# nikopj/FluxMPI.jl

Hardware: AMD Instinct MI355X
Metric: images/sec ResNet50 Lux.jl DDP at 1/2/4/8 MI355X; scaling efficiency (higher is better)
Workload: dtype bf16; 1 GPU; model=ResNet50, global_batch=256, per_gpu_batch=256, image_size=224, parallelism=dp1, optimizer=adam, conv=hybrid, norm=fused, memory_format=channels_last, backend=rccl, miopen_find=True, hip_graph=False, tunableop=False, kernel_choices=shipped, loss_finite=True, communicate=False

## Files before the change

csrc/api.h:

```cpp
#pragma once
#include <hip/hip_runtime.h>
#include <cstdint>
#include <vector>

namespace fluxmpi {

void mt_copy(const std::vector<uintptr_t>& src, const std::vector<uintptr_t>& dst,
             const std::vector<int64_t>& numel, int in_dtype, int out_dtype, float scale,
             hipStream_t stream);

void mt_fill(const std::vector<uintptr_t>& dst, const std::vector<int64_t>& numel, int dtype,
             float value, hipStream_t stream);

void mt_sumsq(const std::vector<uintptr_t>& src, const std::vector<int64_t>& numel, int dtype,
              float* out, hipStream_t stream);

struct AdamHyper {
  float lr, beta1, beta2, eps;
  float bc1, bc2;
  float weight_decay;
  float grad_scale;
  const float* dev;
  const float* dev_gscale;
  const void* tscale = nullptr;
// ... 123 lines not shown
                  int wdtype, hipStream_t stream, bool colsum);

struct GemmProblem {
  const void* a;
  const void* b;
  void* c;
  int64_t lda, ldb, ldc, M, N, K;
  bool a_kmajor, b_kmajor;
  int mode, splits;
  const float* a_scale;
  const float* a_shift;
  const float* b_scale;
  const float* b_shift;
  float* stats;
  int tile_m, tile_n;
  int nbuf;
  const void* res;
  int64_t ldr;
  const void* bnb_x;
  const float* bnb_w;
  const float* bnb_b;
  const float* bnb_mean;
  const float* bnb_inv;
  const uint8_t* bnb_mask;
  int bnb_rm;
  int conv_h = 0, conv_w = 0, conv_c = 0;
  int engine = 0;
  const uint8_t* res_mask = nullptr;
  int res_sub_h = 0, res_sub_w = 0;
  int a_sub_h = 0, a_sub_w = 0;
  int conv_s = 1;
};
void gemm_bf16(const GemmProblem& g, hipStream_t stream);
bool gemm_glds_supported(const GemmProblem& g);
void gemm_glds(const GemmProblem& g, hipStream_t stream);
void gemm_wgrad(const void* a, const void* b, float* ws, int64_t lda, int64_t ldb, int64_t M, int64_t N, int64_t K,
                int splits, int conv_h, int conv_w, int conv_c, hipStream_t stream, int variant = 0, int b_sub = 0);
void transpose_filters(const std::vector<uintptr_t>& src, const std::vector<uintptr_t>& dst,
                       const std::vector<int>& co, const std::vector<int>& ci, const std::vector<int>& taps,
                       hipStream_t stream);
void gemm_splitk_reduce(const float* ws, int splits, int64_t n, void* out, int out_dtype, hipStream_t stream);
void gemm_splitk_reduce_seg(const float* ws, int splits, int64_t n, int64_t seg, void* out0, void* out1, void* out2,
                            int out_dtype, hipStream_t stream);
bool wgrad256_supported(int64_t M, int64_t N, int64_t K, int64_t lda, int64_t ldb);
int wgrad256_actual_splits(int64_t K, int splits);
void wgrad256_set_variant(int v);
void gemm_wgrad256(const void* a, const void* b, float* ws, int64_t lda, int64_t ldb, int64_t M, int64_t N, int64_t K,
                   int splits, hipStream_t stream);
bool gemm_nt_supported(int64_t M, int64_t N, int64_t K, int64_t lda, int64_t ldb, int64_t ldc);
bool gemm_nt_conv_supported(int64_t pixels, int64_t C, int64_t Cout);
int gemm_nt_colpart_rows(int64_t M);
void gemm_nt_set_split(int min_ktiles);
int gemm_nt_get_split();
void gemm_nt(const void* a, const void* b, void* c, void* c2, const void* bias, int bias_f32, const void* h,
             float* colpart, float* stats, int64_t lda, int64_t ldb, int64_t ldc, int64_t M, int64_t N, int64_t K,
             int epi, hipStream_t stream);
void gemm_nt_conv(const void* x, const void* w, void* y, float* stats, int64_t nimg, int H, int W, int C,
                  int64_t Cout, int epi, hipStream_t stream, const void* residual = nullptr);
bool linear_bwd_supported(int64_t M, int64_t N, int64_t K, int64_t ldy, int64_t ldx, int64_t ldw, int64_t lddx);
int linear_bwd_splits(int64_t M, int64_t N, int64_t K, int splits);
void linear_bwd(const void* dy, const void* x, const void* w, void* dx, float* ws, int64_t M, int64_t N, int64_t K,
                int64_t ldy, int64_t ldx, int64_t ldw, int64_t lddx, int splits, int dg_first, hipStream_t stream);
bool conv_c3_supported(int64_t N, int H, int W, int stride, int Cout);
int64_t conv_c3_wgrad_blocks(int64_t N, int H, int W, int stride);
void conv_c3_fwd(const void* x, const void* w_pairs, void* y, int64_t N, int H, int W, int stride, int Cout,
                 hipStream_t stream);
// ... 57 lines not shown
```

csrc/kernels/batchnorm.hip:

```cpp
#include <cstdlib>
#include <initializer_list>
#include <stdexcept>
#include <string>

#include "../api.h"
#include "common.h"

namespace fluxmpi {
namespace {

constexpr int kThreads = 256;
constexpr int kMaxC = 2048;

template <typename T>
struct V8 {
  T v[8];
};

template <typename T>
__device__ __forceinline__ void ld8f(const T* __restrict__ p, float (&f)[8]) {
  T t[8];
  load8(p, t);
#pragma unroll
  for (int j = 0; j < 8; ++j) f[j] = static_cast<float>(t[j]);
}

template <typename T>
__device__ __forceinline__ void st8f(T* __restrict__ p, const float (&f)[8]) {
  T t[8];
#pragma unroll
  for (int j = 0; j < 8; ++j) t[j] = static_cast<T>(f[j]);
  store8(p, t);
}

__device__ __forceinline__ void ld8ch(const float* __restrict__ p, int c0, float (&v)[8]) {
  const float4 a = *reinterpret_cast<const float4*>(p + c0);
  const float4 b = *reinterpret_cast<const float4*>(p + c0 + 4);
  v[0] = a.x; v[1] = a.y; v[2] = a.z; v[3] = a.w;
// ... 445 lines not shown
      for (int u = 0; u < U; ++u)
#pragma unroll
        for (int j = 0; j < 8; ++j) {
          float dd = static_cast<float>(d[u][j]);
          const float xf = static_cast<float>(xv[u][j]);
          if (RM == 1) dd = static_cast<float>(yv[u][j]) > 0.f ? dd : 0.f;
          if (RM == 2) dd = fmaf(xf, sc[j], sh[j]) > 0.f ? dd : 0.f;
          if (RM == 3) dd = (mb[u] >> j) & 1u ? dd : 0.f;
          s[j] += dd;
          q[j] = fmaf(dd, (xf - mu[j]) * is[j], q[j]);
        }
    }
    for (; r < end; r += g.rpi) {
      const int64_t off = r * C + c8 * 8;
      float d[8], xv[8], yv[8];
      ld8f(dy + off, d);
      ld8f(x + off, xv);
      if (RM == 1) ld8f(y + off, yv);
      const unsigned mbs = RM == 3 ? mask[off >> 3] : 0u;
#pragma unroll
      for (int j = 0; j < 8; ++j) {
        float dd = d[j];
        if (RM == 1) dd = yv[j] > 0.f ? dd : 0.f;
        if (RM == 2) dd = fmaf(xv[j], sc[j], sh[j]) > 0.f ? dd : 0.f;
        if (RM == 3) dd = (mbs >> j) & 1u ? dd : 0.f;
        s[j] += dd;
        q[j] = fmaf(dd, (xv[j] - mu[j]) * is[j], q[j]);
      }
    }
  }
  block_reduce<DET>(s, q, g.cv, g.rpi, C, acc, smem);
}

struct DxCoef {
  float a, b, d, sh;
};

__device__ __forceinline__ DxCoef dx_coef(int c, const float* __restrict__ w, const float* __restrict__ bias,
                                          const float* __restrict__ smean, const float* __restrict__ sinv,
                                          const float* __restrict__ dw, const float* __restrict__ db, float inv_n) {
  const float iv = sinv[c], m = smean[c];
  const float sc = (w ? w[c] : 1.f) * iv;
  const float k2 = db[c] * inv_n, k3 = dw[c] * inv_n;
  DxCoef k;
  k.a = sc;
  k.b = -sc * iv * k3;
  k.d = sc * (m * iv * k3 - k2);
  k.sh = fmaf(-m, sc, bias ? bias[c] : 0.f);
  return k;
}

template <typename T, int RM, bool DRES>
__device__ __forceinline__ void dx_vec(float (&d)[8], float (&xv)[8], const float (&yv)[8], unsigned mbs,
                                       const DxCoef* k) {
#pragma unroll
  for (int j = 0; j < 8; ++j) {
    float dd = d[j];
    if (RM == 1) dd = yv[j] > 0.f ? dd : 0.f;
    if (RM == 3) dd = (mbs >> j) & 1u ? dd : 0.f;
    if (RM == 2) dd = fmaf(xv[j], k[j].a, k[j].sh) > 0.f ? dd : 0.f;
    d[j] = dd;
    xv[j] = fmaf(k[j].a, dd, fmaf(k[j].b, xv[j], k[j].d));
  }
}

template <typename T, int RM, bool DRES, bool FIXED, int U = 2>
__global__ __launch_bounds__(kThreads) void bn_bwd_dx_kernel(const T* __restrict__ dy, const T* __restrict__ x,
                                                             const T* __restrict__ y,
                                                             const uint8_t* __restrict__ mask,
                                                             const float* __restrict__ w,
                                                             const float* __restrict__ bias,
                                                             const float* __restrict__ smean,
                                                             const float* __restrict__ sinv,
                                                             const float* __restrict__ dw,
                                                             const float* __restrict__ db, T* __restrict__ dx,
                                                             T* __restrict__ dres, int64_t rows, int C,
                                                             int64_t nvec) {
  extern __shared__ __attribute__((aligned(16))) DxCoef ksm[];
  const float inv_n = 1.f / static_cast<float>(rows);
  DxCoef rk[8];
  if (FIXED) {
    const int c0 = (threadIdx.x % (C / 8)) * 8;
    float iv[8], m[8], ww[8], bb[8], kdb[8], kdw[8];
    ld8ch(sinv, c0, iv);
    ld8ch(smean, c0, m);
    ld8ch(db, c0, kdb);
    ld8ch(dw, c0, kdw);
    ld8ch(w ? w : smean, c0, ww);
    ld8ch(bias ? bias : smean, c0, bb);
#pragma unroll
    for (int j = 0; j < 8; ++j) {
      const float sc = (w ? ww[j] : 1.f) * iv[j];
      const float k2 = kdb[j] * inv_n, k3 = kdw[j] * inv_n;
      rk[j].a = sc;
      rk[j].b = -sc * iv[j] * k3;
      rk[j].d = sc * (m[j] * iv[j] * k3 - k2);
      rk[j].sh = fmaf(-m[j], sc, bias ? bb[j] : 0.f);
    }
  } else {
    for (int c = threadIdx.x; c < C; c += kThreads) ksm[c] = dx_coef(c, w, bias, smean, sinv, dw, db, inv_n);
    __syncthreads();
  }
  const int64_t stride = static_cast<int64_t>(gridDim.x) * kThreads;
  int64_t v = static_cast<int64_t>(blockIdx.x) * kThreads + threadIdx.x;
  for (; v + (U - 1) * stride < nvec; v += U * stride) {
    float d[U][8], xv[U][8], yv[U][8];
    unsigned mb[U];
#pragma unroll
    for (int u = 0; u < U; ++u) {
      const int64_t vu = v + u * stride;
      ld8f(dy + vu * 8, d[u]);
      ld8f(x + vu * 8, xv[u]);
      if (RM == 1) ld8f(y + vu * 8, yv[u]);
      mb[u] = RM == 3 ? mask[vu] : 0u;
    }
    __builtin_amdgcn_sched_barrier(0);
#pragma unroll
    for (int u = 0; u < U; ++u) {
      const int64_t vu = v + u * stride;
      dx_vec<T, RM, DRES>(d[u], xv[u], yv[u], mb[u], FIXED ? rk : ksm + (vu * 8) % C);
      st8f(dx + vu * 8, xv[u]);
      if (DRES) st8f(dres + vu * 8, d[u]);
    }
  }
  for (; v < nvec; v += stride) {
    float d0[8], x0[8], y0[8];
    ld8f(dy + v * 8, d0);
    ld8f(x + v * 8, x0);
    if (RM == 1) ld8f(y + v * 8, y0);
    const unsigned m0 = RM == 3 ? mask[v] : 0u;
    dx_vec<T, RM, DRES>(d0, x0, y0, m0, FIXED ? rk : ksm + (v * 8) % C);
// ... 376 lines not shown
                       int stats_ready, int dtype, hipStream_t s, int64_t* nbt) {
  check(C);
  if (!stats_ready)
    dispatch_float(dtype, kBadDtype, [&](auto tag) { stats_t<typename decltype(tag)::type>(x, ws, rows, C, s); });
  finalize_fwd(ws, rows, C, momentum, eps, sm, si, rm, rv, w, b, scale, shift, nbt, s);
}

void bn_apply(const void* x, void* y, const void* res, const float* w, const float* b, const float* sm,
              const float* si, int64_t rows, int64_t C, int relu, uint8_t* mask, int dtype, hipStream_t s) {
  check(C);
  check_aligned({w, b, sm, si});
  dispatch_float(dtype, kBadDtype, [&](auto tag) {
    norm_t<typename decltype(tag)::type>(x, y, res, w, b, sm, si, rows, C, 0.f, 1, relu, mask, s);
  });
}

void bn_fwd_infer(const void* x, void* y, const void* residual, const float* weight, const float* bias,
                  const float* running_mean, const float* running_var, int64_t rows, int64_t C, float eps, int relu,
                  int dtype, hipStream_t stream) {
  check(C);
  check_aligned({weight, bias, running_mean, running_var});
  dispatch_float(dtype, kBadDtype, [&](auto tag) {
    norm_t<typename decltype(tag)::type>(x, y, residual, weight, bias, running_mean, running_var, rows, C, eps, 0, relu,
                                         nullptr, stream);
  });
}

void bn_bwd(const void* dy, const void* x, const void* y, const uint8_t* relu_mask, const float* weight,
            const float* bias, const float* save_mean,
            const float* save_invstd, void* dx, void* dres, float* dweight, float* dbias, float* workspace,
            int64_t rows, int64_t C, int relu, int dtype, hipStream_t stream, int stats_ready) {
  check(C);
  check_aligned({weight, bias, save_mean, save_invstd, dweight, dbias});
  const int rm = relu_mode(relu, y, relu_mask);
  dispatch_float(dtype, kBadDtype, [&](auto tag) {
    using T = typename decltype(tag)::type;
    if (!stats_ready)
      bwd_reduce_t<T, false>(dy, x, y, relu_mask, weight, bias, save_mean, save_invstd, workspace, rows, C, rm, stream);
    bn_finalize_bwd(workspace, C, dweight, dbias, stream);
    dx_t<T>(dy, x, y, relu_mask, weight, bias, save_mean, save_invstd, dweight, dbias, dx, dres, rows, rows, C, rm,
            stream);
  });
}

size_t bn_sync_workspace_floats(int64_t rows, int64_t C) {
  check(C);
  return static_cast<size_t>(det_geometry(rows, C).blocks) * 2 * static_cast<size_t>(C);
}

void bn_sync_stats(const void* x, float* part, float* msg, int64_t rows, int64_t C, int dtype, hipStream_t stream,
                   float* save_mean, float* save_invstd, float* running_mean, float* running_var, float momentum,
                   float eps, int64_t* nbt) {
  check(C);
  check_rows(rows);
  check_aligned({msg, save_mean, save_invstd});
  const Geo g = det_geometry(rows, C);
  dispatch_float(dtype, kBadSyncDtype, [&](auto tag) {
    using T = typename decltype(tag)::type;
    bn_stats_kernel<T, true><<<g.blocks, kThreads, reduce_smem(g, C), stream>>>(static_cast<const T*>(x), rows, (int)C,
                                                                                g, part);
  });
  FLUXMPI_HIP_CHECK(hipGetLastError());
  bn_sync_fold_fwd_kernel<<<fold_blocks(C), kFoldCh * kFoldGroups, 0, stream>>>(
      part, g.blocks, (int)C, rows, msg, momentum, eps, save_mean, save_invstd, running_mean, running_var, nbt);
  FLUXMPI_HIP_CHECK(hipGetLastError());
}

void bn_sync_finalize_fwd(const float* msg, float* running_mean, float* running_var, float* save_mean,
                          float* save_invstd, int64_t C, float momentum, float eps, hipStream_t stream,
                          int64_t* nbt) {
  check(C);
  check_aligned({save_mean, save_invstd});
// ... 46 lines not shown
```

csrc/kernels/gemm.hip:

```cpp
#include <cstdlib>
#include <stdexcept>
#include <string>

#include "../api.h"
#include "common.h"

namespace fluxmpi {
namespace {

typedef __bf16 bf16x8 __attribute__((ext_vector_type(8)));
typedef __bf16 bf16x4 __attribute__((ext_vector_type(4)));
typedef float f32x4 __attribute__((ext_vector_type(4)));

constexpr int kThreads = 256;
constexpr int BK = 32;
constexpr int kShards = 64;

struct GemmArgs {
  const bf16* a;
  const bf16* b;
  void* c;
  int64_t lda, ldb, ldc;
  int64_t M, N, K;
  int64_t k_per_split;
// ... 497 lines not shown
    o[3] = static_cast<TO>(r.w);
  }
}

template <typename TO>
__global__ __launch_bounds__(kThreads) void sumall_kernel(const float* __restrict__ ws, int S, TO* __restrict__ out) {
  float acc = 0.f;
  for (int i = threadIdx.x; i < S; i += kThreads) acc += ws[i];
  __shared__ float red[kThreads / 64];
  const float w = wave_sum_dpp(acc);
  if ((threadIdx.x & 63) == 0) red[threadIdx.x >> 6] = w;
  __syncthreads();
  if (threadIdx.x == 0) {
    float t = 0.f;
#pragma unroll
    for (int i = 0; i < kThreads / 64; ++i) t += red[i];
    out[0] = static_cast<TO>(t);
  }
}

template <int BM, int BN, bool AK, bool BKM, int NBUF, bool EX = false, bool CONV = false>
void launch(const GemmArgs& a0, int splits, hipStream_t s) {
  GemmArgs a = a0;
  a.tiles_m = static_cast<int>((a.M + BM - 1) / BM);
  a.tiles_n = static_cast<int>((a.N + BN - 1) / BN);
  dim3 grid(a.tiles_m * a.tiles_n, 1, splits);
  gemm_kernel<BM, BN, AK, BKM, NBUF, EX, CONV><<<grid, kThreads, 0, s>>>(a);
  FLUXMPI_HIP_CHECK(hipGetLastError());
}

}

void gemm_bf16(const GemmProblem& g, hipStream_t stream) {
  const bool glds_only = g.res_mask != nullptr || g.res_sub_h > 0 || g.a_sub_h > 0 || g.conv_s == 2 || g.conv_s >= 16;
  if (glds_only && !gemm_glds_supported(g))
    throw std::runtime_error("gemm_bf16: a masked / subsampled residual or a subsampled A needs the LDS-DMA kernel");
  if (g.engine >= 2 || glds_only || (g.engine == 0 && g.a_scale == nullptr && gemm_glds_supported(g))) {
    gemm_glds(g, stream);
    return;
  }
  if ((g.a_kmajor || g.b_kmajor) && g.K % 8 != 0) throw std::runtime_error("gemm_bf16: K-major operands need K % 8 == 0");
  if ((g.a_kmajor ? g.lda : g.lda) % 8 != 0 || g.ldb % 8 != 0)
    throw std::runtime_error("gemm_bf16: leading dimensions must be multiples of 8");
  if (g.mode == 1 && g.stats == nullptr) throw std::runtime_error("gemm_bf16: stats buffer required");
  if ((g.a_scale != nullptr) && !g.a_kmajor) throw std::runtime_error("gemm_bf16: A affine needs K-major A");
  if ((g.b_scale != nullptr) && g.b_kmajor) throw std::runtime_error("gemm_bf16: B affine needs N-major B");
  GemmArgs a{};
  a.a = static_cast<const bf16*>(g.a);
  a.b = static_cast<const bf16*>(g.b);
  a.c = g.c;
  a.lda = g.lda; a.ldb = g.ldb; a.ldc = g.ldc;
  a.M = g.M; a.N = g.N; a.K = g.K;
  int splits = g.splits < 1 ? 1 : g.splits;
  int64_t kps = ((g.K + BK - 1) / BK + splits - 1) / splits * BK;
  splits = static_cast<int>((g.K + kps - 1) / kps);
  a.k_per_split = kps;
  a.a_scale = g.a_scale; a.a_shift = g.a_shift;
  a.b_scale = g.b_scale; a.b_shift = g.b_shift;
  a.stats = g.stats;
  a.mode = g.mode;
  a.res = static_cast<const bf16*>(g.res);
  a.ldr = g.ldr;
  a.bnb_x = static_cast<const bf16*>(g.bnb_x);
  a.bnb_w = g.bnb_w;
  a.bnb_b = g.bnb_b;
  a.bnb_mean = g.bnb_mean;
// ... 118 lines not shown
```

fluxmpi_amd/_build.py:

```python
from __future__ import annotations

import concurrent.futures as cf
import glob
import os
import shutil
import subprocess
import sys
import sysconfig

ROOT = os.path.dirname(os.path.dirname(os.path.abspath(__file__)))
CSRC = os.path.join(ROOT, "csrc")
BUILD = os.path.join(ROOT, "build", "native")
ROCM = os.environ.get("ROCM_PATH", "/opt/rocm")
ARCH = os.environ.get("FLUXMPI_ARCH", "gfx950")


def _ext_suffix() -> str:
    return sysconfig.get_config_var("EXT_SUFFIX") or ".so"


def output_path() -> str:
    return os.path.join(ROOT, "fluxmpi_amd", "_C" + _ext_suffix())


def _sources() -> list[str]:
    srcs = sorted(glob.glob(os.path.join(CSRC, "**", "*.hip"), recursive=True))
    srcs += sorted(glob.glob(os.path.join(CSRC, "**", "*.cpp"), recursive=True))
    return srcs


def _headers() -> list[str]:
    return sorted(glob.glob(os.path.join(CSRC, "**", "*.h"), recursive=True))


def _torch_lib() -> str:
    import importlib.util

    spec = importlib.util.find_spec("torch")
    return os.path.join(os.path.dirname(spec.origin), "lib")


def _tool(name: str) -> str:
    for cand in (os.path.join(ROCM, "bin", name), os.path.join(ROCM, "llvm", "bin", name), shutil.which(name)):
        if cand and os.path.exists(cand):
            return cand
    raise FileNotFoundError(f"{name} not found (ROCM_PATH={ROCM})")


def _obj_for(src: str) -> str:
    rel = os.path.relpath(src, CSRC).replace(os.sep, "__")
    return os.path.join(BUILD, rel + ".o")


_NO_SLP = ["-fno-slp-vectorize"]
EXTRA_FLAGS = {f: _NO_SLP for f in ("gemm_nt.hip", "attention.hip", "gemm_glds.hip", "gemm.hip", "conv3x3n.hip",
                                        "wgrad3x3n.hip", "linbwd.hip")}


def _compile_cmd(src: str, obj: str) -> list[str]:
    import pybind11

    common = ["-O3", "-fPIC", "-std=c++17", "-I", CSRC, "-Wall", "-Wno-unused-function",
              "-Wno-unused-variable", "-Wno-unused-but-set-variable"]
    if src.endswith(".hip"):
        return [_tool("hipcc"), f"--offload-arch={ARCH}", "-c", src, "-o", obj, *common,
                "-munsafe-fp-atomics", *EXTRA_FLAGS.get(os.path.basename(src), [])]
    inc = [f"-I{pybind11.get_include()}", f"-I{sysconfig.get_paths()['include']}", f"-I{ROCM}/include"]
    return [_tool("amdclang++"), "-D__HIP_PLATFORM_AMD__=1", "-c", src, "-o", obj, *common, *inc,
            "-fvisibility=hidden"]


def _stale(obj: str, deps: list[str]) -> bool:
    if not os.path.exists(obj):
        return True
    t = os.path.getmtime(obj)
    return any(os.path.getmtime(d) > t for d in deps)


def build(force: bool = False, verbose: bool = False, jobs: int | None = None) -> str:
    os.makedirs(BUILD, exist_ok=True)
    headers = _headers()
    srcs = _sources()
    out = output_path()
    jobs = jobs or min(8, os.cpu_count() or 4)

    todo = [(s, _obj_for(s)) for s in srcs if force or _stale(_obj_for(s), [s, *headers])]

    def run(cmd):
        if verbose:
            print(" ".join(cmd), flush=True)
        r = subprocess.run(cmd, capture_output=True, text=True)
        if r.returncode != 0:
            raise RuntimeError(f"command failed ({r.returncode}): {' '.join(cmd)}\n{r.stdout}\n{r.stderr}")
        if verbose and (r.stderr.strip()):
            print(r.stderr, file=sys.stderr)
        return r

    with cf.ThreadPoolExecutor(max_workers=jobs) as ex:
        list(ex.map(lambda so: run(_compile_cmd(*so)), todo))

    objs = [_obj_for(s) for s in srcs]
    if force or todo or _stale(out, objs):
        tl = _torch_lib()
        cmd = [_tool("hipcc"), f"--offload-arch={ARCH}", "-shared", "-fPIC", "-o", out + ".tmp", *objs,
               f"-L{ROCM}/lib", "-lamdhip64", f"-L{tl}", "-l:librccl.so", f"-Wl,-rpath,{tl}",
               f"-Wl,-rpath,{ROCM}/lib"]
        run(cmd)
        os.replace(out + ".tmp", out)
    return out


if __name__ == "__main__":
    p = build(force="--force" in sys.argv, verbose=True)
    print(p)
```

fluxmpi_amd/models/resnet.py:

```python
from __future__ import annotations

import os

import torch
import torch.nn as nn
import torch.nn.functional as F

from ..ops.linear import Linear

STEM = os.environ.get("FLUXMPI_STEM", "ours")


class Conv1x1(nn.Module):

    def __init__(self, cin: int, cout: int, stride: int = 1):
        super().__init__()
        self.stride = stride
        self.weight = nn.Parameter(torch.empty(cout, cin, 1, 1))
        nn.init.kaiming_normal_(self.weight, mode="fan_out", nonlinearity="relu")

    def forward(self, x):
        if self.stride != 1:
            x = x[:, :, ::self.stride, ::self.stride]
        n, c, h, w = x.shape
# ... 84 lines not shown
                    a1 = fb.bn_from_stats(c1, self.bn1, relu=True, stats_ready=True) if o1 else \
                        self.bn1(c1, relu=True)
                else:
                    c1 = fb.conv1x1_stats(x, self.conv1.weight, link)
                    a1 = fb.bn_from_stats(c1, self.bn1, relu=True)
                cds = None
                if self.downsample is None:
                    identity = x
                elif fused_ds:
                    ds = self.downsample
                    dual = fb.dual_bn_ok(x, ds[0].out_channels, self.bn3, ds[1])
                    ds_stats = dual and fb.ds_forward_is_ours(x, ds[0].weight, ds[0].stride[0])
                    identity = fb.conv1x1_downsample(x, ds[0].weight, ds[0].stride[0],
                                                     link if isinstance(link, fb.SideGradLink) else None,
                                                     ours_stats=ds_stats)
                    if dual:
                        cds, identity = identity, None
                    else:
                        identity = ds[1](identity)
                else:
                    identity = self.downsample(x)
                if self.hybrid:
                    if fb.conv3x3_supported(a1, self.conv2):
                        ours = fb.conv3x3_forward_is_ours(a1, self.conv2.weight)
                        c2 = fb.conv3x3(a1, self.conv2.weight, with_stats=True)
                        a2 = fb.bn_from_stats(c2, self.bn2, relu=True, stats_ready=ours)
                    elif fb.conv3x3_s2_supported(a1, self.conv2):
                        ours = fb.conv3x3_s2_forward_is_ours(a1, self.conv2.weight)
                        c2 = fb.conv3x3_s2(a1, self.conv2.weight, with_stats=ours)
                        a2 = fb.bn_from_stats(c2, self.bn2, relu=True, stats_ready=ours)
                    else:
                        a2 = self.bn2(self.conv2(a1), relu=True)
                    o3 = fb.conv1x1_forward_is_ours(a2, self.conv3.weight)
                    c3 = fb.conv1x1_hybrid(a2, self.conv3.weight, None, ours_stats=o3)
                else:
                    c2 = fb.conv3x3(a1, self.conv2.weight) if fb.conv3x3_supported(a1, self.conv2) else self.conv2(a1)
                    c3 = fb.bn_relu_conv1x1(c2, self.bn2, self.conv3.weight)
                if cds is not None:
                    out = fb.dual_bn_relu(c3, self.bn3, cds, self.downsample[1],
                                          stats_ready=o3 if self.hybrid else True, ds_stats_ready=ds_stats)
                elif self.hybrid and not o3:
                    out = self.bn3(c3, relu=True, residual=identity, link=link if self.downsample is None else None)
                elif self.hybrid:
                    out = fb.bn_from_stats(c3, self.bn3, relu=True, residual=identity, stats_ready=True,
                                           link=link if self.downsample is None else None)
                else:
                    out = fb.bn_from_stats(c3, self.bn3, relu=True, residual=identity,
                                           link=link if self.downsample is None else None)
                return out
        identity = x if self.downsample is None else self.downsample(x)
        if self.fused:
            out = self.bn1(self.conv1(x), relu=True)
            out = self.bn2(self.conv2(out), relu=True)
            return self.bn3(self.conv3(out), relu=True, residual=identity)
        out = F.relu(self.bn1(self.conv1(x)))
        out = F.relu(self.bn2(self.conv2(out)))
        out = self.bn3(self.conv3(out))
        return F.relu(out + identity)


class ResNet(nn.Module):
    def __init__(self, layers=(3, 4, 6, 3), num_classes=1000, conv_impl="gemm", norm="torch", zero_init_residual=False):
        super().__init__()
        if conv_impl in ("fused", "hybrid"):
            if norm == "sync":
                raise ValueError(f"norm='sync' cannot be combined with conv_impl={conv_impl!r}: those blocks and the "
# ... 79 lines not shown
```

fluxmpi_amd/ops/fused_block.py:

```python
from __future__ import annotations

import torch

from . import _ext
from . import graddst
from .batchnorm import BNStatsLink, GradLink, SideGradLink, _dual_workspace, _link_workspace, _workspace, bn_counter
from . import gemm as G
from . import gemm_nt as _NT
from . import groupnorm as _GN
from .conv_choice import (_DGRAD_CHOICE, _DS_CHOICE, _FWD1_CHOICE, _FWD_CHOICE, _FWD_ENGINE, _S2_CHOICE,
                          _WG_CHOICE, FWD_ENGINES, choices_frozen, dump_choices, freeze_choices,
                          load_choice_lines, load_choices, no_measure as _no_measure, stats_choice,
                          time_us as _time_us, w256_ok as _w256_ok, w3n_configs, wgrad_best)
from .gemm import conv1x1_dgrad, conv1x1_wgrad, conv3x3_dgrad, conv3x3_fwd, gemm, note_filter
from .multi_tensor import DTYPE_CODE


CONV3X3 = "ours"
CONV1X1 = "ours"
DUAL_BN = True
DS_FWD = "ours"
DS_WGRAD = True
S2_FWD = True


def _stream(t):
    return torch.cuda.current_stream(t.device).cuda_stream


def _p(t):
    return t.data_ptr() if t is not None else 0


# ... 246 lines not shown
                            float(eps), int(stats_ready), DTYPE_CODE[x.dtype], _stream(x), _p(nbt))
        res = None
        if residual is not None:
            res = residual if residual.is_contiguous(memory_format=torch.channels_last) else \
                residual.contiguous(memory_format=torch.channels_last)
        y = torch.empty_like(x)
        mask = torch.empty(x.numel() // 8, device=x.device, dtype=torch.uint8) if (relu and res is not None) \
            else None
        C.bn_apply(x.data_ptr(), y.data_ptr(), _p(res), w32.data_ptr(), b32.data_ptr(), mean.data_ptr(),
                   inv.data_ptr(), rows, ch, int(relu), _p(mask), DTYPE_CODE[x.dtype], _stream(x))
        ctx.relu, ctx.has_res, ctx.wdtype = relu, residual is not None, weight.dtype
        ctx.params = (weight, bias)
        ctx.link = link if residual is not None else None
        ctx.bnlink = bnlink
        if bnlink is not None:
            bnlink.bind(x, mask, w32, b32, mean, inv, relu)
        ctx.save_for_backward(x, mask, w32, b32, mean, inv)
        return y

    @staticmethod
    def backward(ctx, dy):
        x, mask, w32, b32, mean, inv = ctx.saved_tensors
        if not dy.is_contiguous(memory_format=torch.channels_last):
            dy = dy.contiguous(memory_format=torch.channels_last)
        ready = ctx.bnlink is not None and ctx.bnlink.ready
        hand_masked = ctx.link is not None and ctx.link.masked and mask is not None and ctx.relu
        dx, dres, dw, db = _bn_bwd(dy, x, mask, w32, b32, mean, inv, ctx.relu, ctx.has_res and not hand_masked,
                                   ready, ctx.params)
        if ctx.bnlink is not None:
            ctx.bnlink.release()
        if ctx.link is not None:
            ctx.link.grad, dres = ((dy, mask) if hand_masked else dres), None
        return dx, dw.to(ctx.wdtype), db.to(ctx.wdtype), dres, None, None, None, None, None, None, None, None, None


class _DualBN(torch.autograd.Function):

    @staticmethod
    def forward(ctx, c3, w, b, rm, rv, mom, eps, nbt, stats_ready, cds, w2, b2, rm2, rv2, mom2, eps2, nbt2,
                ds_ready=False):
        C = _ext.get(required=True)
        cl = torch.channels_last
        c3 = c3 if c3.is_contiguous(memory_format=cl) else c3.contiguous(memory_format=cl)
        cds = cds if cds.is_contiguous(memory_format=cl) else cds.contiguous(memory_format=cl)
        ch = c3.shape[1]
        rows = c3.numel() // ch
        f32 = dict(device=c3.device, dtype=torch.float32)
        w32, b32, w232, b232 = w.float(), b.float(), w2.float(), b2.float()
        mean, inv, mean2, inv2 = (torch.empty(ch, **f32) for _ in range(4))
        ws, code, st = _workspace(c3), DTYPE_CODE[c3.dtype], _stream(c3)
        C.bn_stats_finalize(c3.data_ptr(), w32.data_ptr(), b32.data_ptr(), _p(rm), _p(rv), mean.data_ptr(),
                            inv.data_ptr(), 0, 0, ws.data_ptr(), rows, ch, float(mom), float(eps), int(stats_ready),
                            code, st, _p(nbt))
        ws2 = _dual_workspace(c3) if ds_ready else ws
        C.bn_stats_finalize(cds.data_ptr(), w232.data_ptr(), b232.data_ptr(), _p(rm2), _p(rv2), mean2.data_ptr(),
                            inv2.data_ptr(), 0, 0, ws2.data_ptr(), rows, ch, float(mom2), float(eps2), int(ds_ready),
                            code, st, _p(nbt2))
        y = torch.empty_like(c3)
        mask = torch.empty(c3.numel() // 8, device=c3.device, dtype=torch.uint8)
        C.bn_apply_dual(c3.data_ptr(), cds.data_ptr(), y.data_ptr(), w32.data_ptr(), b32.data_ptr(), mean.data_ptr(),
                        inv.data_ptr(), w232.data_ptr(), b232.data_ptr(), mean2.data_ptr(), inv2.data_ptr(), rows, ch,
                        mask.data_ptr(), code, st)
        ctx.wdtypes = (w.dtype, w2.dtype)
        ctx.params = (w, b, w2, b2)
        ctx.save_for_backward(c3, cds, mask, w32, mean, inv, w232, mean2, inv2)
        return y
# ... 321 lines not shown
```

Measured before the change: 12490 images/s.

## Fuse bn3 backward dx with conv3 dgrad and wgrad in one kernel

Adds a fused HIP kernel for the conv3 (1x1, 64->256) plus bn3 plus ReLU tail of the bottleneck block's first stage. The backward pass computes the BN dx in registers, stages it in LDS, and runs both the data-gradient GEMM and the weight-gradient GEMM from that tile, writing per-block slabs that are then reduced. The aim is to avoid writing the bn dx tensor to HBM and reading it back twice. The cost is an extra split-K reduce, a specialised shape-only path, and a build check that fails compilation if the kernel spills to scratch.

```diff
diff --git a/csrc/api.h b/csrc/api.h
--- a/csrc/api.h
+++ b/csrc/api.h
@@ -179,6 +179,7 @@
   int conv_s = 1;
 };
 void gemm_bf16(const GemmProblem& g, hipStream_t stream);
+void conv3bn3_bwd(const GemmProblem& g, hipStream_t stream);
 bool gemm_glds_supported(const GemmProblem& g);
 void gemm_glds(const GemmProblem& g, hipStream_t stream);
 void gemm_wgrad(const void* a, const void* b, float* ws, int64_t lda, int64_t ldb, int64_t M, int64_t N, int64_t K,
diff --git a/csrc/kernels/batchnorm.hip b/csrc/kernels/batchnorm.hip
--- a/csrc/kernels/batchnorm.hip
+++ b/csrc/kernels/batchnorm.hip
@@ -4,6 +4,7 @@
 #include <string>
 
 #include "../api.h"
+#include "bn_dx.h"
 #include "common.h"
 
 namespace fluxmpi {
@@ -515,38 +516,6 @@
   block_reduce<DET>(s, q, g.cv, g.rpi, C, acc, smem);
 }
 
-struct DxCoef {
-  float a, b, d, sh;
-};
-
-__device__ __forceinline__ DxCoef dx_coef(int c, const float* __restrict__ w, const float* __restrict__ bias,
-                                          const float* __restrict__ smean, const float* __restrict__ sinv,
-                                          const float* __restrict__ dw, const float* __restrict__ db, float inv_n) {
-  const float iv = sinv[c], m = smean[c];
-  const float sc = (w ? w[c] : 1.f) * iv;
-  const float k2 = db[c] * inv_n, k3 = dw[c] * inv_n;
-  DxCoef k;
-  k.a = sc;
-  k.b = -sc * iv * k3;
-  k.d = sc * (m * iv * k3 - k2);
-  k.sh = fmaf(-m, sc, bias ? bias[c] : 0.f);
-  return k;
-}
-
-template <typename T, int RM, bool DRES>
-__device__ __forceinline__ void dx_vec(float (&d)[8], float (&xv)[8], const float (&yv)[8], unsigned mbs,
-                                       const DxCoef* k) {
-#pragma unroll
-  for (int j = 0; j < 8; ++j) {
-    float dd = d[j];
-    if (RM == 1) dd = yv[j] > 0.f ? dd : 0.f;
-    if (RM == 3) dd = (mbs >> j) & 1u ? dd : 0.f;
-    if (RM == 2) dd = fmaf(xv[j], k[j].a, k[j].sh) > 0.f ? dd : 0.f;
-    d[j] = dd;
-    xv[j] = fmaf(k[j].a, dd, fmaf(k[j].b, xv[j], k[j].d));
-  }
-}
-
 template <typename T, int RM, bool DRES, bool FIXED, int U = 2>
 __global__ __launch_bounds__(kThreads) void bn_bwd_dx_kernel(const T* __restrict__ dy, const T* __restrict__ x,
                                                              const T* __restrict__ y,
@@ -572,14 +541,8 @@
     ld8ch(w ? w : smean, c0, ww);
     ld8ch(bias ? bias : smean, c0, bb);
 #pragma unroll
-    for (int j = 0; j < 8; ++j) {
-      const float sc = (w ? ww[j] : 1.f) * iv[j];
-      const float k2 = kdb[j] * inv_n, k3 = kdw[j] * inv_n;
-      rk[j].a = sc;
-      rk[j].b = -sc * iv[j] * k3;
-      rk[j].d = sc * (m[j] * iv[j] * k3 - k2);
-      rk[j].sh = fmaf(-m[j], sc, bias ? bb[j] : 0.f);
-    }
+    for (int j = 0; j < 8; ++j)
+      rk[j] = dx_coef_of(w != nullptr, ww[j], bias != nullptr, bb[j], m[j], iv[j], kdw[j], kdb[j], inv_n);
   } else {
     for (int c = threadIdx.x; c < C; c += kThreads) ksm[c] = dx_coef(c, w, bias, smean, sinv, dw, db, inv_n);
     __syncthreads();
@@ -1022,12 +985,15 @@
             int64_t rows, int64_t C, int relu, int dtype, hipStream_t stream, int stats_ready) {
   check(C);
   check_aligned({weight, bias, save_mean, save_invstd, dweight, dbias});
+  if (dx == nullptr && dres != nullptr)
+    throw std::runtime_error("fused batchnorm: bn_bwd without a dx (reduce and finalize only) writes no dres either");
   const int rm = relu_mode(relu, y, relu_mask);
   dispatch_float(dtype, kBadDtype, [&](auto tag) {
     using T = typename decltype(tag)::type;
     if (!stats_ready)
       bwd_reduce_t<T, false>(dy, x, y, relu_mask, weight, bias, save_mean, save_invstd, workspace, rows, C, rm, stream);
     bn_finalize_bwd(workspace, C, dweight, dbias, stream);
+    if (dx == nullptr) return;
     dx_t<T>(dy, x, y, relu_mask, weight, bias, save_mean, save_invstd, dweight, dbias, dx, dres, rows, rows, C, rm,
             stream);
   });
diff --git a/csrc/kernels/bn_dx.h b/csrc/kernels/bn_dx.h
--- /dev/null
+++ b/csrc/kernels/bn_dx.h
@@ -0,0 +1,44 @@
+#pragma once
+#include <hip/hip_runtime.h>
+
+namespace fluxmpi {
+
+struct DxCoef {
+  float a, b, d, sh;
+};
+
+__device__ __forceinline__ DxCoef dx_coef_of(bool has_w, float wv, bool has_bias, float bv, float m, float iv,
+                                             float dwv, float dbv, float inv_n) {
+  const float sc = (has_w ? wv : 1.f) * iv;
+  const float k2 = dbv * inv_n, k3 = dwv * inv_n;
+  DxCoef k;
+  k.a = sc;
+  k.b = -sc * iv * k3;
+  k.d = sc * (m * iv * k3 - k2);
+  k.sh = fmaf(-m, sc, has_bias ? bv : 0.f);
+  return k;
+}
+
+__device__ __forceinline__ DxCoef dx_coef(int c, const float* __restrict__ w, const float* __restrict__ bias,
+                                          const float* __restrict__ smean, const float* __restrict__ sinv,
+                                          const float* __restrict__ dw, const float* __restrict__ db, float inv_n) {
+  const float iv = sinv[c], m = smean[c];
+  const float wv = w ? w[c] : 1.f, dwv = dw[c], dbv = db[c], bv = bias ? bias[c] : 0.f;
+  return dx_coef_of(true, wv, true, bv, m, iv, dwv, dbv, inv_n);
+}
+
+template <typename T, int RM, bool DRES>
+__device__ __forceinline__ void dx_vec(float (&d)[8], float (&xv)[8], const float (&yv)[8], unsigned mbs,
+                                       const DxCoef* k) {
+#pragma unroll
+  for (int j = 0; j < 8; ++j) {
+    float dd = d[j];
+    if (RM == 1) dd = yv[j] > 0.f ? dd : 0.f;
+    if (RM == 3) dd = (mbs >> j) & 1u ? dd : 0.f;
+    if (RM == 2) dd = fmaf(xv[j], k[j].a, k[j].sh) > 0.f ? dd : 0.f;
+    d[j] = dd;
+    xv[j] = fmaf(k[j].a, dd, fmaf(k[j].b, xv[j], k[j].d));
+  }
+}
+
+}
diff --git a/csrc/kernels/conv3bn3_bwd.hip b/csrc/kernels/conv3bn3_bwd.hip
--- /dev/null
+++ b/csrc/kernels/conv3bn3_bwd.hip
@@ -0,0 +1,262 @@
+#include <mutex>
+#include <stdexcept>
+#include <string>
+#include <vector>
+
+#include "../api.h"
+#include "bn_dx.h"
+#include "common.h"
+
+namespace fluxmpi {
+namespace {
+
+typedef __bf16 bf16x8 __attribute__((ext_vector_type(8)));
+typedef __bf16 bf16x4 __attribute__((ext_vector_type(4)));
+typedef float f32x4 __attribute__((ext_vector_type(4)));
+
+constexpr int kThreads = 256;
+constexpr int kCo = 256, kCi = 64;
+constexpr int kTP = 32;
+constexpr int kLdT = kCo + 8;
+constexpr int kLdS = kCi + 8;
+constexpr int kLdW = kCi;
+constexpr int kWBytes = kCo * kLdW * 2, kTBytes = kTP * kLdT * 2, kABytes = kTP * kLdS * 2;
+constexpr int kKBytes = 3 * kCo * static_cast<int>(sizeof(float));
+constexpr int kSmem = kWBytes + kTBytes + kABytes + kKBytes;
+static_assert(kThreads == kCo, "one lane per channel computes the coefficients");
+constexpr int kRpi = kThreads / (kCo / 8);
+constexpr int kRows = kTP / kRpi;
+constexpr int kAv = kTP * (kCi / 8) / kThreads;
+
+struct C3Args {
+  const bf16* dy;
+  const bf16* x3;
+  const uint8_t* mask;
+  const float* w;
+  const float* mean;
+  const float* inv;
+  const float* sum_dy;
+  const float* sum_dy_xhat;
+  const bf16* a2;
+  const bf16* wt;
+  bf16* d_a2;
+  float* ws;
+  int64_t P;
+};
+
+__device__ __forceinline__ bf16x8 frag_tr(const bf16* __restrict__ img, int ld, int k0, int c0) {
+  const int l = threadIdx.x & 63;
+  const int g = l >> 4, li = l & 15, q = li >> 2, p = li & 3;
+  const bf16* a0 = img + (k0 + 8 * g + q) * ld + c0 + 4 * p;
+  const bf16* a1 = a0 + 4 * ld;
+  typedef short short4v __attribute__((ext_vector_type(4)));
+  typedef __attribute__((address_space(3))) short4v lds_short4v;
+  short4v lo = __builtin_amdgcn_ds_read_tr16_b64_v4i16((lds_short4v*)(a0));
+  short4v hi = __builtin_amdgcn_ds_read_tr16_b64_v4i16((lds_short4v*)(a1));
+  bf16x8 out;
+  __builtin_memcpy(&out, &lo, 8);
+  __builtin_memcpy(reinterpret_cast<char*>(&out) + 8, &hi, 8);
+  return out;
+}
+
+__device__ __forceinline__ void ld4(const float* __restrict__ p, float* v) {
+  const float4 a = *reinterpret_cast<const float4*>(p);
+  v[0] = a.x; v[1] = a.y; v[2] = a.z; v[3] = a.w;
+}
+
+__global__ __launch_bounds__(kThreads, 2) void conv3bn3_bwd_kernel(C3Args p) {
+  extern __shared__ __attribute__((aligned(16))) char smem[];
+  bf16* wimg = reinterpret_cast<bf16*>(smem);
+  bf16* tile = reinterpret_cast<bf16*>(smem + kWBytes);
+  bf16* atile = reinterpret_cast<bf16*>(smem + kWBytes + kTBytes);
+  float* ksm = reinterpret_cast<float*>(smem + kWBytes + kTBytes + kABytes);
+  const int t = threadIdx.x;
+  const int wave = __builtin_amdgcn_readfirstlane(t >> 6), lane = t & 63;
+  const int vec = t & 31, r0 = t >> 5;
+  const int arow = t >> 3, avec = t & 7;
+  const int64_t ntiles = (p.P + kTP - 1) / kTP;
+
+#pragma unroll
+  for (int i = 0; i < kCo * kCi / 8 / kThreads; ++i) {
+    const int v = t + i * kThreads;
+    const uint4 q = reinterpret_cast<const uint4*>(p.wt)[v];
+    *reinterpret_cast<uint4*>(wimg + (v >> 3) * kLdW + (v & 7) * 8) = q;
+  }
+  {
+    const DxCoef k = dx_coef(t, p.w, nullptr, p.mean, p.inv, p.sum_dy_xhat, p.sum_dy, 1.f / static_cast<float>(p.P));
+    const int slot = ((t >> 2) & 1) * 128 + (t >> 3) * 4 + (t & 3);
+    ksm[slot] = k.a;
+    ksm[kCo + slot] = k.b;
+    ksm[2 * kCo + slot] = k.d;
+  }
+  __syncthreads();
+
+  bf16x8 wf[kCo / 32];
+#pragma unroll
+  for (int ks = 0; ks < kCo / 32; ++ks) wf[ks] = frag_tr(wimg, kLdW, 32 * ks, 16 * wave);
+
+  uint4 qd[kRows], qx[kRows], qa[kAv];
+  unsigned mb[kRows];
+  auto issue = [&](int64_t tl) {
+    const int64_t p0 = tl * kTP;
+    const int nr = p.P - p0 < kTP ? static_cast<int>(p.P - p0) : kTP;
+    const bf16* dyb = p.dy + p0 * kCo;
+    const bf16* x3b = p.x3 + p0 * kCo;
+    const uint8_t* mkb = p.mask + p0 * (kCo / 8);
+#pragma unroll
+    for (int i = 0; i < kRows; ++i) {
+      const int r = r0 + kRpi * i < nr ? r0 + kRpi * i : nr - 1;
+      const unsigned v = static_cast<unsigned>(r) * (kCo / 8) + vec;
+      qd[i] = reinterpret_cast<const uint4*>(dyb)[v];
+      qx[i] = reinterpret_cast<const uint4*>(x3b)[v];
+      mb[i] = mkb[v];
+    }
+#pragma unroll
+    for (int i = 0; i < kAv; ++i) {
+      const int ra = arow + 32 * i < nr ? arow + 32 * i : nr - 1;
+      qa[i] = reinterpret_cast<const uint4*>(p.a2 + p0 * kCi)[static_cast<unsigned>(ra) * (kCi / 8) + avec];
+    }
+  };
+
+  f32x4 acc[4][4];
+#pragma unroll
+  for (int i = 0; i < 4; ++i)
+#pragma unroll
+    for (int j = 0; j < 4; ++j) acc[i][j] = f32x4{0.f, 0.f, 0.f, 0.f};
+
+  int64_t tl = blockIdx.x;
+  if (tl < ntiles) issue(tl);
+  for (; tl < ntiles; tl += gridDim.x) {
+    const int64_t p0 = tl * kTP;
+    int opq = 0;
+    asm volatile("" : "+v"(opq));
+    const float4* kl = reinterpret_cast<const float4*>(ksm + opq) + vec;
+    DxCoef rk[8];
+#pragma unroll
+    for (int hf = 0; hf < 2; ++hf) {
+      const float4 ka = kl[hf * 32], kb = kl[64 + hf * 32], kd = kl[128 + hf * 32];
+      rk[4 * hf + 0] = DxCoef{ka.x, kb.x, kd.x, 0.f};
+      rk[4 * hf + 1] = DxCoef{ka.y, kb.y, kd.y, 0.f};
+      rk[4 * hf + 2] = DxCoef{ka.z, kb.z, kd.z, 0.f};
+      rk[4 * hf + 3] = DxCoef{ka.w, kb.w, kd.w, 0.f};
+    }
+#pragma unroll
+    for (int i = 0; i < kRows; ++i) {
+      bf16 td[8], tx[8];
+      __builtin_memcpy(td, &qd[i], 16);
+      __builtin_memcpy(tx, &qx[i], 16);
+      float d[8], xv[8];
+#pragma unroll
+      for (int j = 0; j < 8; ++j) {
+        d[j] = static_cast<float>(td[j]);
+        xv[j] = static_cast<float>(tx[j]);
+      }
+      dx_vec<bf16, 3, false>(d, xv, d, mb[i], rk);
+      const bool ok = p0 + r0 + kRpi * i < p.P;
+      bf16x8 o;
+#pragma unroll
+      for (int j = 0; j < 8; ++j) o[j] = ok ? static_cast<bf16>(xv[j]) : static_cast<bf16>(0.f);
+      *reinterpret_cast<bf16x8*>(tile + (r0 + kRpi * i) * kLdT + vec * 8) = o;
+      __builtin_amdgcn_sched_barrier(0);
+    }
+#pragma unroll
+    for (int i = 0; i < kAv; ++i)
+      *reinterpret_cast<uint4*>(atile + (arow + 32 * i) * kLdS + avec * 8) =
+          p0 + arow + 32 * i < p.P ? qa[i] : uint4{0u, 0u, 0u, 0u};
+    __syncthreads();
+    if (tl + gridDim.x < ntiles) issue(tl + gridDim.x);
+
+    {
+      f32x4 da[kTP / 16];
+#pragma unroll
+      for (int i = 0; i < kTP / 16; ++i) da[i] = f32x4{0.f, 0.f, 0.f, 0.f};
+      const bf16* brow = tile + (lane & 15) * kLdT + 8 * (lane >> 4);
+#pragma unroll
+      for (int ks = 0; ks < kCo / 32; ++ks) {
+#pragma unroll
+        for (int i = 0; i < kTP / 16; ++i) {
+          const bf16x8 fb = *reinterpret_cast<const bf16x8*>(brow + 16 * i * kLdT + 32 * ks);
+          da[i] = __builtin_amdgcn_mfma_f32_16x16x32_bf16(wf[ks], fb, da[i], 0, 0, 0);
+        }
+      }
+      bf16* ob = p.d_a2 + p0 * kCi;
+      const unsigned oo = static_cast<unsigned>(lane & 15) * kCi + 16 * wave + 4 * (lane >> 4);
+#pragma unroll
+      for (int i = 0; i < kTP / 16; ++i) {
+        if (p0 + 16 * i + (lane & 15) < p.P) {
+          bf16x4 o;
+#pragma unroll
+          for (int r = 0; r < 4; ++r) o[r] = static_cast<bf16>(da[i][r]);
+          *reinterpret_cast<bf16x4*>(ob + oo + 16 * i * kCi) = o;
+        }
+      }
+    }
+#pragma unroll
+    for (int kh = 0; kh < kTP / 32; ++kh) {
+      bf16x8 fb[4];
+#pragma unroll
+      for (int j = 0; j < 4; ++j) fb[j] = frag_tr(atile, kLdS, 32 * kh, 16 * j);
+#pragma unroll
+      for (int i = 0; i < 4; ++i) {
+        const bf16x8 fa = frag_tr(tile, kLdT, 32 * kh, wave * 64 + 16 * i);
+#pragma unroll
+        for (int j = 0; j < 4; ++j) acc[i][j] = __builtin_amdgcn_mfma_f32_16x16x32_bf16(fa, fb[j], acc[i][j], 0, 0, 0);
+      }
+    }
+    __syncthreads();
+  }
+
+  float* slab = p.ws + static_cast<int64_t>(blockIdx.x) * (kCo * kCi);
+#pragma unroll
+  for (int i = 0; i < 4; ++i)
+#pragma unroll
+    for (int j = 0; j < 4; ++j)
+#pragma unroll
+      for (int r = 0; r < 4; ++r)
+        slab[static_cast<unsigned>((wave * 64 + 16 * i + 4 * (lane >> 4) + r) * kCi + 16 * j + (lane & 15))] = acc[i][j][r];
+}
+
+void allow_lds() {
+  static std::mutex mu;
+  static std::vector<char> done;
+  int dev = 0;
+  FLUXMPI_HIP_CHECK(hipGetDevice(&dev));
+  std::lock_guard<std::mutex> lock(mu);
+  if (static_cast<size_t>(dev) >= done.size()) done.resize(dev + 1, 0);
+  if (done[dev]) return;
+  FLUXMPI_HIP_CHECK(hipFuncSetAttribute(reinterpret_cast<const void*>(&conv3bn3_bwd_kernel),
+                                        hipFuncAttributeMaxDynamicSharedMemorySize, kSmem));
+  done[dev] = 1;
+}
+
+}
+
+void conv3bn3_bwd(const GemmProblem& g, hipStream_t stream) {
+  if (g.N != kCi || g.K != kCo || g.M < 1 || g.lda != kCo || g.ldb != kCi || g.ldc != kCi || g.ldr != kCi ||
+      !g.a_kmajor || g.b_kmajor || g.bnb_rm != 3)
+    throw std::runtime_error("gemm_bf16 mode 4: needs N = 64, K = 256, dense operands (lda = 256, ldb = ldc = ldr = 64), "
+                             "K-major A, N-major B and the 1-bit ReLU mask (bnb_rm = 3); got M=" + std::to_string(g.M) +
+                             ", N=" + std::to_string(g.N) + ", K=" + std::to_string(g.K));
+  if (g.a == nullptr || g.b == nullptr || g.c == nullptr || g.res == nullptr || g.bnb_x == nullptr ||
+      g.bnb_mask == nullptr || g.bnb_mean == nullptr || g.bnb_inv == nullptr || g.a_scale == nullptr ||
+      g.a_shift == nullptr || g.stats == nullptr)
+    throw std::runtime_error("gemm_bf16 mode 4: dy, W, d_a2, a2 (res), x3 (bnb_x), the mask, mean / invstd, the two "
+                             "sums (a_scale / a_shift) and the slab workspace (stats) are all required");
+  uintptr_t bits = 0;
+  for (const void* q : {g.a, g.b, static_cast<const void*>(g.c), g.res, g.bnb_x, static_cast<const void*>(g.bnb_w),
+                        static_cast<const void*>(g.bnb_mean), static_cast<const void*>(g.bnb_inv),
+                        static_cast<const void*>(g.a_scale), static_cast<const void*>(g.a_shift),
+                        static_cast<const void*>(g.stats)})
+    bits |= reinterpret_cast<uintptr_t>(q);
+  if ((bits & 15u) != 0) throw std::runtime_error("gemm_bf16 mode 4: operands must be 16-byte aligned");
+  if (g.splits < 1 || g.splits > 65535)
+    throw std::runtime_error("gemm_bf16 mode 4: splits (the slab count = workgroups) must be in [1, 65535]");
+  allow_lds();
+  C3Args p{static_cast<const bf16*>(g.a), static_cast<const bf16*>(g.bnb_x), g.bnb_mask, g.bnb_w, g.bnb_mean,
+           g.bnb_inv, g.a_scale, g.a_shift, static_cast<const bf16*>(g.res), static_cast<const bf16*>(g.b),
+           static_cast<bf16*>(g.c), g.stats, g.M};
+  conv3bn3_bwd_kernel<<<static_cast<unsigned>(g.splits), kThreads, kSmem, stream>>>(p);
+  FLUXMPI_HIP_CHECK(hipGetLastError());
+}
+
+}
diff --git a/csrc/kernels/gemm.hip b/csrc/kernels/gemm.hip
--- a/csrc/kernels/gemm.hip
+++ b/csrc/kernels/gemm.hip
@@ -553,6 +553,10 @@
 }
 
 void gemm_bf16(const GemmProblem& g, hipStream_t stream) {
+  if (g.mode == 4) {
+    conv3bn3_bwd(g, stream);
+    return;
+  }
   const bool glds_only = g.res_mask != nullptr || g.res_sub_h > 0 || g.a_sub_h > 0 || g.conv_s == 2 || g.conv_s >= 16;
   if (glds_only && !gemm_glds_supported(g))
     throw std::runtime_error("gemm_bf16: a masked / subsampled residual or a subsampled A needs the LDS-DMA kernel");
diff --git a/fluxmpi_amd/_build.py b/fluxmpi_amd/_build.py
--- a/fluxmpi_amd/_build.py
+++ b/fluxmpi_amd/_build.py
@@ -3,6 +3,7 @@
 import concurrent.futures as cf
 import glob
 import os
+import re
 import shutil
 import subprocess
 import sys
@@ -54,7 +55,18 @@
 
 _NO_SLP = ["-fno-slp-vectorize"]
 EXTRA_FLAGS = {f: _NO_SLP for f in ("gemm_nt.hip", "attention.hip", "gemm_glds.hip", "gemm.hip", "conv3x3n.hip",
-                                        "wgrad3x3n.hip", "linbwd.hip")}
+                                        "wgrad3x3n.hip", "linbwd.hip", "conv3bn3_bwd.hip")}
+
+
+NO_SCRATCH = ("conv3bn3_bwd.hip",)
+
+
+def _check_no_scratch(src: str, remarks: str) -> None:
+    sizes = [int(m) for m in re.findall(r"ScratchSize \[bytes/lane\]: (\d+)", remarks)]
+    if not sizes:
+        raise RuntimeError(f"{src}: the compiler printed no kernel resource usage to check for scratch")
+    if any(sizes):
+        raise RuntimeError(f"{src}: a kernel spills to scratch ({max(sizes)} bytes/lane); it must not\n{remarks}")
 
 
 def _compile_cmd(src: str, obj: str) -> list[str]:
@@ -64,7 +76,8 @@
               "-Wno-unused-variable", "-Wno-unused-but-set-variable"]
     if src.endswith(".hip"):
         return [_tool("hipcc"), f"--offload-arch={ARCH}", "-c", src, "-o", obj, *common,
-                "-munsafe-fp-atomics", *EXTRA_FLAGS.get(os.path.basename(src), [])]
+                "-munsafe-fp-atomics", *EXTRA_FLAGS.get(os.path.basename(src), []),
+                *(["-Rpass-analysis=kernel-resource-usage"] if os.path.basename(src) in NO_SCRATCH else [])]
     inc = [f"-I{pybind11.get_include()}", f"-I{sysconfig.get_paths()['include']}", f"-I{ROCM}/include"]
     return [_tool("amdclang++"), "-D__HIP_PLATFORM_AMD__=1", "-c", src, "-o", obj, *common, *inc,
             "-fvisibility=hidden"]
@@ -97,7 +110,16 @@
         return r
 
     with cf.ThreadPoolExecutor(max_workers=jobs) as ex:
-        list(ex.map(lambda so: run(_compile_cmd(*so)), todo))
+        def compile_one(so):
+            r = run(_compile_cmd(*so))
+            if os.path.basename(so[0]) in NO_SCRATCH:
+                try:
+                    _check_no_scratch(so[0], r.stderr)
+                except RuntimeError:
+                    os.remove(so[1])
+                    raise
+
+        list(ex.map(compile_one, todo))
 
     objs = [_obj_for(s) for s in srcs]
     if force or todo or _stale(out, objs):
diff --git a/fluxmpi_amd/models/resnet.py b/fluxmpi_amd/models/resnet.py
--- a/fluxmpi_amd/models/resnet.py
+++ b/fluxmpi_amd/models/resnet.py
@@ -140,6 +140,8 @@
                     else:
                         a2 = self.bn2(self.conv2(a1), relu=True)
                     o3 = fb.conv1x1_forward_is_ours(a2, self.conv3.weight)
+                    if self.downsample is None and fb.conv3bn3_ok(a2, self.conv3, self.bn3, identity, link):
+                        return fb.conv3_bn3_relu(a2, self.conv3, self.bn3, identity, link, ours_fwd=o3)
                     c3 = fb.conv1x1_hybrid(a2, self.conv3.weight, None, ours_stats=o3)
                 else:
                     c2 = fb.conv3x3(a1, self.conv2.weight) if fb.conv3x3_supported(a1, self.conv2) else self.conv2(a1)
diff --git a/fluxmpi_amd/ops/fused_block.py b/fluxmpi_amd/ops/fused_block.py
--- a/fluxmpi_amd/ops/fused_block.py
+++ b/fluxmpi_amd/ops/fused_block.py
@@ -1,4 +1,6 @@
 from __future__ import annotations
+
+import os
 
 import torch
 
@@ -311,6 +313,89 @@
         if ctx.link is not None:
             ctx.link.grad, dres = ((dy, mask) if hand_masked else dres), None
         return dx, dw.to(ctx.wdtype), db.to(ctx.wdtype), dres, None, None, None, None, None, None, None, None, None
+
+
+class _Conv3BN3(torch.autograd.Function):
+
+    @staticmethod
+    def forward(ctx, a2, weight, bn_weight, bn_bias, residual, running_mean, running_var, momentum, eps, nbt, link,
+                ours_fwd):
+        C = _ext.get(required=True)
+        cl = torch.channels_last
+        a2 = a2 if a2.is_contiguous(memory_format=cl) else a2.contiguous(memory_format=cl)
+        res = residual if residual.is_contiguous(memory_format=cl) else residual.contiguous(memory_format=cl)
+        note_filter(weight)
+        ws = _workspace(a2)
+        c3 = _fwd1x1_stats(a2, weight, ws) if ours_fwd else torch.nn.functional.conv2d(a2, weight)
+        ch = c3.shape[1]
+        rows = c3.numel() // ch
+        w32, b32 = bn_weight.float(), bn_bias.float()
+        mean = torch.empty(ch, device=c3.device, dtype=torch.float32)
+        inv = torch.empty_like(mean)
+        C.bn_stats_finalize(c3.data_ptr(), w32.data_ptr(), b32.data_ptr(), _p(running_mean), _p(running_var),
+                            mean.data_ptr(), inv.data_ptr(), 0, 0, ws.data_ptr(), rows, ch, float(momentum),
+                            float(eps), int(ours_fwd), DTYPE_CODE[c3.dtype], _stream(c3), _p(nbt))
+        y = torch.empty_like(c3)
+        mask = torch.empty(c3.numel() // 8, device=c3.device, dtype=torch.uint8)
+        C.bn_apply(c3.data_ptr(), y.data_ptr(), res.data_ptr(), w32.data_ptr(), b32.data_ptr(), mean.data_ptr(),
+                   inv.data_ptr(), rows, ch, 1, mask.data_ptr(), DTYPE_CODE[c3.dtype], _stream(c3))
+        ctx.link, ctx.wdtype, ctx.params = link, bn_weight.dtype, (bn_weight, bn_bias)
+        ctx.save_for_backward(a2, weight, c3, mask, w32, b32, mean, inv)
+        return y
+
+    @staticmethod
+    def backward(ctx, dy):
+        C = _ext.get(required=True)
+        a2, weight, c3, mask, w32, b32, mean, inv = ctx.saved_tensors
+        if not dy.is_contiguous(memory_format=torch.channels_last):
+            dy = dy.contiguous(memory_format=torch.channels_last)
+        n, ci, h, w = a2.shape
+        co, rows = weight.shape[0], n * h * w
+        dev, st = dy.device, _stream(dy)
+        dbw, dbb = _grad_out(ctx.params[0], co, c3), _grad_out(ctx.params[1], co, c3)
+        C.bn_bwd(dy.data_ptr(), c3.data_ptr(), 0, mask.data_ptr(), w32.data_ptr(), b32.data_ptr(), mean.data_ptr(),
+                 inv.data_ptr(), 0, 0, dbw.data_ptr(), dbb.data_ptr(), _workspace(c3).data_ptr(), rows, co, 1,
+                 DTYPE_CODE[c3.dtype], st, 0)
+        slabs = conv3bn3_slabs(rows, dev)
+        part = torch.empty(slabs, co, ci, device=dev, dtype=torch.float32)
+        d_a2 = _empty_nhwc(n, ci, h, w, a2)
+        gemm(dy, weight, d_a2, M=rows, N=ci, K=co, lda=co, ldb=ci, ldc=ci, a_kmajor=True, b_kmajor=False, mode=4,
+             splits=slabs, a_affine=(dbb, dbw), stats=part, residual=_nhwc2d(a2),
+             bn_bwd=(c3, w32, None, mean, inv, mask, 3))
+        dw = None
+        if ctx.needs_input_grad[1]:
+            with graddst.into(weight):
+                dw = graddst.empty((co, ci), weight.dtype, dev)
+            C.gemm_splitk_reduce(part.data_ptr(), slabs, co * ci, dw.data_ptr(), DTYPE_CODE[dw.dtype], st)
+            dw = dw.view(co, ci, 1, 1)
+        if ctx.link is not None:
+            ctx.link.grad = (dy, mask)
+        return (d_a2, dw, dbw.to(ctx.wdtype), dbb.to(ctx.wdtype), None, None, None, None, None, None, None, None)
+
+
+CONV3BN3 = os.environ.get("FLUXMPI_CONV3BN3", "1") != "0"
+
+
+def conv3bn3_slabs(rows: int, device) -> int:
+    cus = torch.cuda.get_device_properties(device).multi_processor_count
+    return max(1, min(-(-rows // 32), 2 * cus))
+
+
+def conv3bn3_ok(a2, conv, bn, residual, link) -> bool:
+    from .batchnorm import FusedBatchNorm2d
+    wt = conv.weight
+    return (CONV3BN3 and G.ENGINE != 1 and a2.is_cuda and a2.dim() == 4 and a2.dtype == torch.bfloat16
+            and wt.dtype == torch.bfloat16 and tuple(wt.shape) == (256, 64, 1, 1) and wt.is_contiguous()
+            and a2.shape[1] == 64 and a2.numel() // 64 < 2 ** 31 and residual is not None
+            and residual.shape == (a2.shape[0], 256, a2.shape[2], a2.shape[3]) and residual.dtype == a2.dtype
+            and (link.masked if link is not None else not (residual.requires_grad and torch.is_grad_enabled()))
+            and isinstance(bn, FusedBatchNorm2d) and bn.training and bn.affine and bn.track_running_stats)
+
+
+def conv3_bn3_relu(a2, conv, bn, residual, link=None, ours_fwd=True):
+    mom, nbt = bn_counter(bn)
+    return _Conv3BN3.apply(a2, conv.weight, bn.weight, bn.bias, residual, bn.running_mean, bn.running_var, mom,
+                           bn.eps, nbt, link, bool(ours_fwd))
 
 
 class _DualBN(torch.autograd.Function):
```

Result: faster. 12800 images/s, median of 6 (+2.5%).
